# jdm365/SuffixArray

Measured on AMD Instinct MI355X. Metric: sa_build_chars_per_s, higher is better.
Workload: dtype u8 text / u32 narrow keys / u32 suffix indices / i64 output

## Files before the change

suffixarray_amd/csrc/radix_narrow.hpp:

```cpp
#pragma once
#include "radix_sort.hpp"
#include <vector>

namespace sa {

constexpr int NARROW_MAX_PASSES = 6;
constexpr int SEG_ITEMS = 24;

struct SegPlan {
    u32 bstart[RADIX + 1];
    u32 tprefix[RADIX + 1];
    u32 cfirst[NCHUNK + 1];
};

__global__ __launch_bounds__(256) void seg_plan_kernel(const u32* __restrict__ hist_top, u32 tile, SegPlan* __restrict__ plan) {
    __shared__ uint2 s_w[4];
    __shared__ u32 s_tp[RADIX + 1];
    const int d = threadIdx.x;
    u32 size = 0;
#pragma unroll
    for (int c = 0; c < NCHUNK; ++c) size += hist_top[c * RADIX + d];
    const u32 tiles = (u32)(((u64)size + tile - 1) / tile);
    uint2 tot;
    const uint2 ex = block_scan_excl<4>(make_uint2(size, tiles), make_uint2(0, 0), ScanSum{}, s_w, &tot);
// ... 796 lines not shown
    template <typename K>
    int persist_grid(K kernel, int block, int slot, u32 nsub, u32* grid) {
        if (!local_grid[slot]) {
            int dev = 0, cus = 0, per_cu = 0;
            SA_HIP_CHECK(hipGetDevice(&dev));
            SA_HIP_CHECK(hipDeviceGetAttribute(&cus, hipDeviceAttributeMultiprocessorCount, dev));
            SA_HIP_CHECK(hipOccupancyMaxActiveBlocksPerMultiprocessor(&per_cu, reinterpret_cast<const void*>(kernel), block, 0));
            local_grid[slot] = (u32)((per_cu > 0 ? per_cu : 1) * (cus > 0 ? cus : 1));
        }
        const u32 g = local_grid_force ? local_grid_force : local_grid[slot];
        *grid = g < nsub ? g : nsub;
        return 0;
    }
    bool split_flags_done = false;
    int split_items = 28;
    static size_t hist_bytes() { return (size_t)NARROW_MAX_PASSES * RADIX * RADIX * sizeof(u32); }
    int init() {
        SA_HIP_CHECK(hipMalloc(&plan, sizeof(SegPlan)));
        SA_HIP_CHECK(hipMalloc(&hist, hist_bytes()));
        SA_HIP_CHECK(hipMalloc(&base, (size_t)RADIX * RADIX * sizeof(u32)));
        SA_HIP_CHECK(hipMalloc(&tickets, (size_t)NARROW_MAX_PASSES * NCHUNK * sizeof(u32)));
        SA_HIP_CHECK(hipMalloc(&map_dev, sizeof(CodeMap)));
        SA_HIP_CHECK(hipMalloc(&split_hist, split_table_bytes()));
        SA_HIP_CHECK(hipMalloc(&split_base, split_table_bytes()));
        SA_HIP_CHECK(hipMalloc(&split_cursor, split_table_bytes()));
        SA_HIP_CHECK(hipMalloc(&top_cursor, (size_t)RADIX * TOP_CURSOR_STRIDE * sizeof(u32)));
        SA_HIP_CHECK(hipMalloc(&split_sub, (split_sub_words() + 16) * sizeof(u32)));
        SA_HIP_CHECK(hipHostMalloc(reinterpret_cast<void**>(&host_word), 64, hipHostMallocDefault));
        if (const char* e = diag_env("SA_HIP_SPLIT")) split_enabled = atoi(e) != 0;
        if (const char* e = diag_env("SA_HIP_TOP_CLAIMS")) top_claims = atoi(e) != 0;
        if (const char* e = diag_env("SA_HIP_LOCAL_BIG")) local_big = atoi(e) != 0;
        if (const char* e = diag_env("SA_HIP_LOCAL_PERSIST")) local_persist = atoi(e) != 0;
        if (const char* e = diag_env("SA_HIP_LOCAL_GRID")) { const int v = atoi(e); local_grid_force = v > 0 ? (u32)v : 0u; }
        if (const char* e = diag_env("SA_HIP_SPLIT_FLAGS")) split_flags = atoi(e) != 0;
        if (const char* e = diag_env("SA_HIP_LOCAL_BINS")) local_bin_bits = (atoi(e) == 11) ? 11 : 12;
        if (const char* e = diag_env("SA_HIP_SPLIT_ITEMS")) { const int v = atoi(e); split_items = (v == 24 || v == 28) ? v : 32; }
        if (const char* e = diag_env("SA_HIP_SPLIT_CAP")) { const int v = atoi(e); if (v >= 64 && v <= (int)LOCAL_CAP) split_cap = (u32)v; }
        return 0;
    }
    void destroy() {
        if (plan) (void)hipFree(plan);
        if (hist) (void)hipFree(hist);
        if (base) (void)hipFree(base);
        if (tickets) (void)hipFree(tickets);
        if (map_dev) (void)hipFree(map_dev);
        if (split_hist) (void)hipFree(split_hist);
        if (split_base) (void)hipFree(split_base);
        if (split_cursor) (void)hipFree(split_cursor);
        if (top_cursor) (void)hipFree(top_cursor);
        if (split_sub) (void)hipFree(split_sub);
        if (host_word) (void)hipHostFree(host_word);
        map_dev = nullptr;
        plan = nullptr; hist = nullptr; base = nullptr; tickets = nullptr;
        split_hist = split_base = split_sub = split_cursor = top_cursor = nullptr; host_word = nullptr;
    }
};

inline bool narrow_sort_applies(const RadixWorkspace& ws, u64 n, int begin_bit) {
    return ws.block == 512 && begin_bit >= 24 && begin_bit < 56 && n >= (1u << 22) &&
           n / ws.tile() + RADIX + 1 <= ws.max_tiles;
}

struct TextSource {
    const u8* text;
    int b, k0;
};
// ... 88 lines not shown
            a.keys_out32 = reinterpret_cast<u32*>(keysB); a.narrow_shift = begin_bit;
            if ((rc = ws.timer.start(stream, 1))) return rc;
            hipLaunchKernelGGL((radix_onesweep_kernel<512, 0, true>), dim3(g.tiles), dim3(512), 0, stream, a);
            if ((rc = ws.timer.stop(stream, (u64)n * 16u))) return rc;
            ws.pass_records += n; ws.pass_bytes += (u64)n * 16u; ws.passes += 1;
        }
    }
    const u32 seg_tile_n = 512u * SEG_ITEMS;
    const u32 flat_max = n / seg_tile_n + 1 + RADIX;
    const u32 split_tile_n = 512u * (u32)nw.split_items;
    const u32 split_flat_max = n / split_tile_n + 1 + RADIX;
    hipLaunchKernelGGL(seg_plan_kernel, dim3(1), dim3(256), 0, stream, ws.hist(0), try_split ? split_tile_n : seg_tile_n, nw.plan);
    nw.split_used = false;
    nw.split_flags_done = false;
    nw.split_max_seen = 0;
    if (try_split) {
        const int hb = (lo_bits - LOCAL_BIN_BITS < SPLIT_BITS) ? lo_bits - LOCAL_BIN_BITS : SPLIT_BITS;
        SA_HIP_CHECK(hipMemsetAsync(nw.split_hist, 0, NarrowWorkspace::split_table_bytes(), stream));
        SA_HIP_CHECK(hipMemsetAsync(nw.split_levels_dev(), 0, 16 * sizeof(u32), stream));
        const u32 tpb = 4;
        if (nw.split_items == 32)
            hipLaunchKernelGGL((split_hist_kernel<512, 32>), dim3(div_up(split_flat_max, tpb)), dim3(512), 0, stream,
                               reinterpret_cast<const u32*>(keysB), nw.plan, lo_bits - hb, (1u << hb) - 1u, nw.split_hist, tpb);
        else if (nw.split_items == 28)
            hipLaunchKernelGGL((split_hist_kernel<512, 28>), dim3(div_up(split_flat_max, tpb)), dim3(512), 0, stream,
                               reinterpret_cast<const u32*>(keysB), nw.plan, lo_bits - hb, (1u << hb) - 1u, nw.split_hist, tpb);
        else
            hipLaunchKernelGGL((split_hist_kernel<512, 24>), dim3(div_up(split_flat_max, tpb)), dim3(512), 0, stream,
                               reinterpret_cast<const u32*>(keysB), nw.plan, lo_bits - hb, (1u << hb) - 1u, nw.split_hist, tpb);
        hipLaunchKernelGGL(split_levels_kernel, dim3(RADIX), dim3(SPLIT_NB), 0, stream, (const u32*)nw.split_hist, hb, nw.split_levels_dev());
        SA_HIP_CHECK(hipMemcpyAsync(nw.host_word, nw.split_levels_dev(), 16 * sizeof(u32), hipMemcpyDeviceToHost, stream));
        SA_HIP_CHECK(hipStreamSynchronize(stream));
        int rb = -1;
        bool big = nw.local_big;
        if (!big)
            for (int k = 1; k <= hb; ++k)
                if (nw.host_word[k] <= nw.split_cap) { rb = k; break; }
        if (rb < 0 && nw.split_cap == LOCAL_CAP) {
            for (int k = 1; k <= hb; ++k)
                if (nw.host_word[k] <= LOCAL_CAP_BIG && lo_bits - k >= 12) { rb = k; big = true; break; }
            if (rb < 0) big = false;
        }
        nw.split_max_seen = nw.host_word[rb > 0 ? rb : hb];
        if (rb > 0) {
            const int rest_bits = lo_bits - rb;
            const int dshift = lo_bits - rb;
            const u32 dmask = (1u << rb) - 1u;
            hipLaunchKernelGGL(split_scan_kernel, dim3(RADIX), dim3(SPLIT_NB), 0, stream, (const u32*)nw.split_hist, nw.plan, hb, rb,
                               nw.split_base, nw.split_sub);
            SA_HIP_CHECK(hipMemsetAsync(nw.split_cursor, 0, NarrowWorkspace::split_table_bytes(), stream));
            if (++ws.epoch >= (1u << 30)) {
                SA_HIP_CHECK(hipMemsetAsync(ws.status, 0, (size_t)ws.max_tiles * RADIX * sizeof(u64), stream));
                ws.epoch = 1;
            }
            SplitPassArgs a;
            a.keys_in = reinterpret_cast<const u32*>(keysB); a.vals_in = valsB;
            a.keys_out = reinterpret_cast<u32*>(keysA); a.vals_out = valsA;
            a.plan = nw.plan; a.shift = dshift; a.mask = dmask; a.digit_base = nw.split_base;
            a.ticket = nw.tickets; a.cursor = nw.split_cursor;
            if ((rc = ws.timer.start(stream, 2))) return rc;
            if (nw.split_items == 32) hipLaunchKernelGGL((seg_split_kernel<512, 32>), dim3(split_flat_max), dim3(512), 0, stream, a);
            else if (nw.split_items == 28) hipLaunchKernelGGL((seg_split_kernel<512, 28>), dim3(split_flat_max), dim3(512), 0, stream, a);
            else hipLaunchKernelGGL((seg_split_kernel<512, 24>), dim3(split_flat_max), dim3(512), 0, stream, a);
            if ((rc = ws.timer.stop(stream, (u64)n * 16u))) return rc;
            ws.pass_records += n; ws.pass_bytes += (u64)n * 16u; ws.passes += 1;
            LocalArgs l;
            l.keys_in = reinterpret_cast<const u32*>(keysA); l.vals_in = valsA;
            l.keys_out = reinterpret_cast<u32*>(keysB); l.vals_out = valsB; l.vals_out64 = vals_res64;
            l.sub = nw.split_sub;
            const int bb = (big || (rest_bits >= 12 && nw.local_bin_bits == 12)) ? 12 : 11;
            l.bin_shift = rest_bits - bb;
            l.dstat = ws.dstat;
            const u64 local_bytes = (u64)n * 16u + (vals_res64 ? (u64)n * 8u : 0u);
            nw.split_flags_done = false;
            l.dir = DirArgs{}; l.counts = nullptr; l.lite = LiteArgs{}; l.lo_shift = begin_bit; l.rb = rb; l.n = n;
            bool with_flags = false;
            if (nw.split_flags && flags_req && flags_req->prepare) {
                const int fr = flags_req->prepare(flags_req->ctx, (u32)RADIX << rb, &l);
                if (fr < 0) return fr;
                with_flags = (fr == 0) && l.dir.dir && l.dir.dbits >= 8 + rb && l.dir.dbits - 8 - rb <= bb && l.dir.dbits - 8 <= lo_bits;
            }
            if ((rc = ws.timer.start(stream, 3))) return rc;
            const u32 nsub = (u32)RADIX << rb;
            const dim3 lgrid(nsub), lblock(big ? LOCAL_BLOCK_BIG : LOCAL_BLOCK);
            if (nw.local_persist) {
                const int slot = big ? (with_flags ? 0 : 1) : 2 + (with_flags ? 0 : 1) + (bb == 12 ? 0 : 2);
                u32 pg = 0;
                auto go = [&](auto kernel) -> int {
                    if ((rc = nw.persist_grid(kernel, (int)lblock.x, slot, nsub, &pg))) return rc;
                    hipLaunchKernelGGL(kernel, dim3(pg), lblock, 0, stream, l, (const u32*)nw.split_sub, nsub, nw.tickets + NCHUNK, LOCAL_RUN);
                    return 0;
                };
                if (big) rc = with_flags ? go(local_persist_kernel<12, true, LOCAL_BLOCK_BIG>) : go(local_persist_kernel<12, false, LOCAL_BLOCK_BIG>);
                else if (with_flags) rc = (bb == 12) ? go(local_persist_kernel<12, true>) : go(local_persist_kernel<11, true>);
                else rc = (bb == 12) ? go(local_persist_kernel<12, false>) : go(local_persist_kernel<11, false>);
                if (rc) return rc;
            } else if (big) {
                if (with_flags) hipLaunchKernelGGL((local_finish_kernel<12, true, LOCAL_BLOCK_BIG>), lgrid, lblock, 0, stream, l);
                else hipLaunchKernelGGL((local_finish_kernel<12, false, LOCAL_BLOCK_BIG>), lgrid, lblock, 0, stream, l);
            } else if (with_flags) {
                if (bb == 12) hipLaunchKernelGGL((local_finish_kernel<12, true>), lgrid, lblock, 0, stream, l);
                else hipLaunchKernelGGL((local_finish_kernel<11, true>), lgrid, lblock, 0, stream, l);
            } else {
                if (bb == 12) hipLaunchKernelGGL((local_finish_kernel<12, false>), lgrid, lblock, 0, stream, l);
                else hipLaunchKernelGGL((local_finish_kernel<11, false>), lgrid, lblock, 0, stream, l);
            }
            nw.split_flags_done = with_flags;
            nw.split_big = big;
            if ((rc = ws.timer.stop(stream, local_bytes))) return rc;
            ws.pass_records += n; ws.pass_bytes += local_bytes; ws.passes += 1;
            SA_HIP_CHECK(hipGetLastError());
            if (diag_env("SA_HIP_SPLIT_DEBUG")) {
                const u32 nsub = (u32)RADIX << rb;
                std::vector<u32> sub(nsub + 1), k1(n), k2(n), v2(n), bst(RADIX + 1);
                SA_HIP_CHECK(hipStreamSynchronize(stream));
                SA_HIP_CHECK(hipMemcpy(sub.data(), nw.split_sub, (size_t)(nsub + 1) * 4, hipMemcpyDeviceToHost));
                SA_HIP_CHECK(hipMemcpy(k1.data(), keysA, (size_t)n * 4, hipMemcpyDeviceToHost));
                SA_HIP_CHECK(hipMemcpy(k2.data(), keysB, (size_t)n * 4, hipMemcpyDeviceToHost));
                SA_HIP_CHECK(hipMemcpy(v2.data(), valsB, (size_t)n * 4, hipMemcpyDeviceToHost));
                SA_HIP_CHECK(hipMemcpy(bst.data(), nw.plan->bstart, (size_t)(RADIX + 1) * 4, hipMemcpyDeviceToHost));
                u64 bad_sub = 0, bad_split = 0, bad_sorted = 0, bad_mono = 0;
                u32 first_split = ~0u, first_sorted = ~0u;
                for (u32 i = 0; i < nsub; ++i) {
                    if (sub[i] > sub[i + 1] || sub[i + 1] > n) { ++bad_mono; continue; }
                    if ((i & (((u32)1 << rb) - 1)) == 0 && sub[i] != bst[i >> rb]) ++bad_sub;
                    for (u32 j = sub[i]; j < sub[i + 1]; ++j) {
                        if (((k1[j] >> dshift) & dmask) != (i & dmask)) { ++bad_split; if (first_split == ~0u) first_split = j; }
                        if (j > sub[i] && (k2[j - 1] > k2[j] || (k2[j - 1] == k2[j] && v2[j - 1] >= v2[j]))) { ++bad_sorted; if (first_sorted == ~0u) first_sorted = j; }
                    }
                }
                fprintf(stderr, "[sa_hip] split debug: n=%u rb=%d hb=%d nsub=%u sub[0]=%u sub[last]=%u | table: %llu not monotone, %llu off the bucket starts | split pass: %llu records in the wrong group (first %u) | local pass: %llu out of order (first %u)\n",
                        n, rb, hb, nsub, sub[0], sub[nsub], (unsigned long long)bad_mono, (unsigned long long)bad_sub, (unsigned long long)bad_split, first_split,
                        (unsigned long long)bad_sorted, first_sorted);
            }
            nw.split_used = true;
            nw.split_rb = rb;
            *keys_res = reinterpret_cast<u64*>(keysB);
            *vals_res = valsB;
            return 0;
        }
    }
    if (optimistic) {
        SA_HIP_CHECK(hipMemsetAsync(ws.tickets(), 0, NCHUNK * sizeof(u32), stream));
        if (++ws.epoch >= (1u << 30)) {
            SA_HIP_CHECK(hipMemsetAsync(ws.status, 0, (size_t)ws.max_tiles * RADIX * sizeof(u64), stream));
            ws.epoch = 1;
        }
        if ((rc = launch_text_top(false))) return rc;
    }
    if (try_split && split_tile_n != seg_tile_n)
        hipLaunchKernelGGL(seg_plan_kernel, dim3(1), dim3(256), 0, stream, ws.hist(0), seg_tile_n, nw.plan);
    SA_HIP_CHECK(hipMemsetAsync(nw.hist, 0, NarrowWorkspace::hist_bytes(), stream));
    {
        const u32 tpb = 4;
        const u32 mask0 = (1u << ((np == 1) ? lo_bits : RADIX_BITS)) - 1u;
// ... 44 lines not shown
```

suffixarray_amd/csrc/radix_split.hpp:

```cpp
#pragma once
#include "flags_common.hpp"

namespace sa {

#ifndef SA_ABL
#define SA_ABL 0
#endif
constexpr int SPLIT_BITS = 10;
constexpr int SPLIT_NB = 1 << SPLIT_BITS;
constexpr u32 LOCAL_CAP = 8192;
constexpr int LOCAL_BLOCK = 512;
constexpr int LOCAL_ITEMS = (int)(LOCAL_CAP / LOCAL_BLOCK);
constexpr u32 LOCAL_CAP_BIG = 16384;
constexpr int LOCAL_BLOCK_BIG = 1024;
constexpr u32 LOCAL_RUN = 8;
constexpr int LOCAL_BIN_BITS = 11;
constexpr int SPLIT_HIST_COPIES = 4;

template <int BLOCK, int ITEMS>
__global__ __launch_bounds__(BLOCK) void split_hist_kernel(const u32* __restrict__ keys, const SegPlan* __restrict__ plan, int shift,
                                                           u32 mask, u32* __restrict__ hist, u32 tiles_per_block) {
    constexpr u32 TILE = BLOCK * ITEMS;
    constexpr int CS = SPLIT_NB + 1;
    __shared__ u32 s_h[SPLIT_HIST_COPIES * CS];
    __shared__ u32 s_t[RADIX + 1];
    for (int i = threadIdx.x; i <= RADIX; i += BLOCK) s_t[i] = plan->tprefix[i];
    for (int i = threadIdx.x; i < SPLIT_HIST_COPIES * CS; i += BLOCK) s_h[i] = 0;
    __syncthreads();
    const u32 F = s_t[RADIX];
    const u32 f_lo = blockIdx.x * tiles_per_block;
    const u32 f_hi = (f_lo + tiles_per_block < F) ? f_lo + tiles_per_block : F;
    if (f_lo >= f_hi) return;
    u32* my = s_h + (threadIdx.x & (SPLIT_HIST_COPIES - 1)) * CS;
    auto flush = [&](u32 bucket) {
        sync_lds();
        for (int d = threadIdx.x; d < SPLIT_NB; d += BLOCK) {
            u32 v = 0;
#pragma unroll
            for (int k = 0; k < SPLIT_HIST_COPIES; ++k) { v += s_h[k * CS + d]; s_h[k * CS + d] = 0; }
            if (v) atomicAdd(&hist[bucket * SPLIT_NB + d], v);
        }
        sync_lds();
    };
    u32 cur = seg_bucket_of(s_t, f_lo);
    for (u32 f = f_lo; f < f_hi; ++f) {
        const u32 b = seg_bucket_of(s_t, f);
        if (b != cur) { flush(cur); cur = b; }
        const u32 start = plan->bstart[b] + ((f - s_t[b]) * TILE);
        const u32 end = plan->bstart[b + 1];
        const u32 len = (end - start) < TILE ? (end - start) : TILE;
        if (len == TILE) {
            u32 k[ITEMS];
#pragma unroll
            for (int j = 0; j < ITEMS; ++j) k[j] = keys[start + j * BLOCK + threadIdx.x];
#pragma unroll
            for (int j = 0; j < ITEMS; ++j) atomicAdd(&my[(k[j] >> shift) & mask], 1u);
        } else {
            for (u32 l = threadIdx.x; l < len; l += BLOCK) atomicAdd(&my[(keys[start + l] >> shift) & mask], 1u);
        }
    }
    flush(cur);
}

__global__ __launch_bounds__(SPLIT_NB) void split_levels_kernel(const u32* __restrict__ hist, int hb, u32* __restrict__ levels) {
    __shared__ u32 s_p[SPLIT_NB + 1];
    __shared__ u32 s_w[SPLIT_NB / WAVE];
    const int b = blockIdx.x, d = threadIdx.x, lane = d & 63, w = d >> 6;
    const u32 c = hist[b * SPLIT_NB + d];
    s_p[d + 1] = block_scan_excl<SPLIT_NB / WAVE>(c, 0u, ScanSum{}, s_w) + c;
    if (d == 0) s_p[0] = 0;
    __syncthreads();
    __shared__ u32 s_lv[SPLIT_BITS + 1][SPLIT_NB / WAVE];
    for (int k = 0; k <= hb; ++k) {
        const int g = hb - k;
        u32 v = 0;
        if (d < (1 << k)) v = s_p[(d + 1) << g] - s_p[d << g];
#pragma unroll
        for (int o = 32; o > 0; o >>= 1) { const u32 t = __shfl_down(v, o); v = t > v ? t : v; }
        if (lane == 0) s_lv[k][w] = v;
    }
    __syncthreads();
    if (d <= hb) {
        u32 v = 0;
        for (int i = 0; i < SPLIT_NB / WAVE; ++i) v = s_lv[d][i] > v ? s_lv[d][i] : v;
        if (v) atomicMax(&levels[d], v);
    }
}

__global__ __launch_bounds__(SPLIT_NB) void split_scan_kernel(const u32* __restrict__ hist, const SegPlan* __restrict__ plan, int hb, int rb,
                                                              u32* __restrict__ base, u32* __restrict__ sub) {
    __shared__ u32 s_w[SPLIT_NB / WAVE];
    const int b = blockIdx.x, d = threadIdx.x;
    const u32 run = plan->bstart[b] + block_scan_excl<SPLIT_NB / WAVE>(hist[b * SPLIT_NB + d], 0u, ScanSum{}, s_w);
    const int g = hb - rb;
    u32 out = 0;
    if (d < (1 << hb) && (d & ((1 << g) - 1)) == 0) {
        out = run;
        sub[((u32)b << rb) + (u32)(d >> g)] = run;
    }
    __shared__ u32 s_o[SPLIT_NB];
    s_o[d] = 0;
    __syncthreads();
    if (d < (1 << hb) && (d & ((1 << g) - 1)) == 0) s_o[d >> g] = out;
    __syncthreads();
    base[b * SPLIT_NB + d] = s_o[d];
    if (d == 0 && b == RADIX - 1) sub[(u32)RADIX << rb] = plan->bstart[RADIX];
}

struct SplitPassArgs {
    const u32* keys_in;
    const u32* vals_in;
    u32* keys_out;
    u32* vals_out;
    const SegPlan* plan;
    int shift;
    u32 mask;
    const u32* digit_base;
    u32* ticket;
    u32* cursor;
};

template <bool FULL, int BLOCK, int ITEMS>
__device__ __forceinline__ void split_tile(const SplitPassArgs& a, const u32 bucket, const u32 start, const u32 tile_n,
                                           u32* s_keys, u32* s_cnt, u32* s_gdelta, u32* s_wsum) {
    static_assert(SPLIT_NB == 2 * BLOCK, "two bins per thread");
    const int tid = threadIdx.x, lane = tid & 63, wave = tid >> 6;
    const u32 woff = (u32)wave * (WAVE * ITEMS) + lane;

    const uint2 dbase = *reinterpret_cast<const uint2*>(a.digit_base + (size_t)bucket * SPLIT_NB + 2 * tid);

    u32 key[ITEMS];
    const u32* kin = a.keys_in + start;
#pragma unroll
    for (int j = 0; j < ITEMS; ++j) {
        const u32 p = woff + j * WAVE;
        key[j] = (FULL || p < tile_n) ? kin[p] : 0u;
    }
    u32 pos[ITEMS];
#pragma unroll
    for (int j = 0; j < ITEMS; ++j) {
        const u32 d = (key[j] >> a.shift) & a.mask;
        pos[j] = atomicAdd(&s_cnt[(FULL || (woff + j * WAVE) < tile_n) ? d : (u32)SPLIT_NB], 1u);
    }
    sync_lds();
// ... 9 lines not shown
    const u32 incl = wave_scan_incl(tot, ScanSum{});
    if (lane == 63) s_wsum[wave] = incl;
    __syncthreads();
    u32 excl = incl - tot;
    for (int i = 0; i < wave; ++i) excl += s_wsum[i];
    *reinterpret_cast<uint2*>(s_cnt + 2 * tid) = make_uint2(excl, excl + c.x);
    __syncthreads();

#pragma unroll
    for (int j = 0; j < ITEMS; ++j) {
        pos[j] += s_cnt[(key[j] >> a.shift) & a.mask];
        if (FULL || (woff + j * WAVE) < tile_n) s_keys[pos[j]] = key[j];
    }
    __syncthreads();

    *reinterpret_cast<uint2*>(s_gdelta + 2 * tid) = make_uint2(dbase.x + claim0 - excl, dbase.y + claim1 - (excl + c.x));
    __syncthreads();

    static_assert(ITEMS % 2 == 0 && BLOCK * ITEMS <= 65536, "positions packed as 16-bit pairs");
    u32 pp[ITEMS / 2];
#pragma unroll
    for (int j = 0; j < ITEMS / 2; ++j) pp[j] = pos[2 * j] | (pos[2 * j + 1] << 16);
    u32 gidx[ITEMS];
#pragma unroll
    for (int k = 0; k < ITEMS; ++k) {
        const u32 p = k * BLOCK + tid;
        if (FULL || p < tile_n) {
            const u32 kk = s_keys[p];
            gidx[k] = s_gdelta[(kk >> a.shift) & a.mask] + p;
            a.keys_out[gidx[k]] = kk;
        }
    }
    u32 val[ITEMS];
    const u32* vin = a.vals_in + start;
#pragma unroll
    for (int j = 0; j < ITEMS; ++j) {
        const u32 p = woff + j * WAVE;
        val[j] = (FULL || p < tile_n) ? vin[p] : 0u;
    }
    __syncthreads();
    u32* s_vals = s_keys;
#pragma unroll
    for (int j = 0; j < ITEMS; ++j)
        if (FULL || (woff + j * WAVE) < tile_n) s_vals[(pp[j >> 1] >> ((j & 1) * 16)) & 0xFFFFu] = val[j];
    __syncthreads();
#pragma unroll
    for (int k = 0; k < ITEMS; ++k) {
        const u32 p = k * BLOCK + tid;
        if (FULL || p < tile_n) a.vals_out[gidx[k]] = s_vals[p];
    }
}

template <int BLOCK, int ITEMS>
__global__ __launch_bounds__(BLOCK, 4) void seg_split_kernel(SplitPassArgs a) {
    constexpr u32 TILE = BLOCK * ITEMS;
    __shared__ __attribute__((aligned(16))) u32 s_keys[TILE];
    __shared__ __attribute__((aligned(16))) u32 s_cnt[SPLIT_NB + 4];
    __shared__ __attribute__((aligned(16))) u32 s_gdelta[SPLIT_NB];
    __shared__ u32 s_wsum[BLOCK / WAVE];
    __shared__ u32 s_t[RADIX + 1];
    __shared__ u32 s_b[RADIX + 1];
    __shared__ u32 s_c[NCHUNK + 1];
    __shared__ u32 s_flat;

    const int tid = threadIdx.x;
    u32 home = 0, t_home = 0;
    if (tid == 0) {
        home = xcc_id();
// ... 6 lines not shown
    if (tid == 0) {
        u32 flat = 0xFFFFFFFFu;
        if (t_home < s_c[home + 1] - s_c[home]) flat = s_c[home] + t_home;
        for (int k = 1; k < NCHUNK && flat == 0xFFFFFFFFu; ++k) {
            const u32 c = (home + k) & (NCHUNK - 1);
            const u32 cnt = s_c[c + 1] - s_c[c];
            if (cnt == 0) continue;
            const u32 t = atomicAdd(&a.ticket[c], 1u);
            if (t < cnt) flat = s_c[c] + t;
        }
        s_flat = flat;
    }
    __syncthreads();
    const u32 flat = s_flat;
    if (flat == 0xFFFFFFFFu) return;
    const u32 bucket = seg_bucket_of(s_t, flat);
    const u32 first_flat = s_t[bucket];
    const u32 start = s_b[bucket] + (flat - first_flat) * TILE;
    const u32 rest = s_b[bucket + 1] - start;
    if (rest >= TILE) split_tile<true, BLOCK, ITEMS>(a, bucket, start, TILE, s_keys, s_cnt, s_gdelta, s_wsum);
    else split_tile<false, BLOCK, ITEMS>(a, bucket, start, rest, s_keys, s_cnt, s_gdelta, s_wsum);
}

struct LocalArgs {
    const u32* keys_in;
    const u32* vals_in;
    u32* keys_out;
    u32* vals_out;
    int64_t* vals_out64;
    const u32* sub;
    int bin_shift;
    DeviceStatus* dstat;
    DirArgs dir;
    uint2* counts;
    LiteArgs lite;
    int lo_shift;
    int rb;
    u32 n;
};

struct LocalFlagsRequest {
    int (*prepare)(void* ctx, u32 nsub, LocalArgs* l) = nullptr;
    void* ctx = nullptr;
};

template <int BB, bool FLAGS, int BLOCK, bool PERSIST, typename Mid>
__device__ __forceinline__ void local_finish_sub(const LocalArgs& a, const u32 sb, const u32 s, const u32 m, u32 (&key)[LOCAL_ITEMS],
                                                 u32 (&val)[LOCAL_ITEMS], u64* s_rec, u32* s_cw, u32* s_wsum, Mid&& mid) {
    constexpr int ITEMS = LOCAL_ITEMS;
    constexpr int NB = 1 << BB, WORDS = NB / 2, WPT = WORDS / BLOCK;
    const int tid = threadIdx.x, lane = tid & 63, wave = tid >> 6;
    const int g2 = FLAGS ? a.dir.dbits - 8 - a.rb : 0;
    const u32 dfirst = FLAGS ? (sb << g2) : 0u;
    const u32 nd = FLAGS ? (1u << g2) : 0u;
// ... 115 lines not shown
                const u32 kn = (u32)__builtin_amdgcn_update_dpp((int)~k, (int)k, 0x101, 0xF, 0xF, false);
                tmask |= (kn == k && p + 1 < m) ? (1u << j) : 0u;
            }
        }
    }
    if (FLAGS) {
        while (tmask) {
            const u32 j = (u32)__builtin_ctz(tmask);
            tmask &= tmask - 1u;
            stage_pair(j * BLOCK + (u32)tid);
        }
    }
}

template <int BLOCK>
__device__ __forceinline__ void local_load(const LocalArgs& a, const u32 s, const u32 m, u32 (&key)[LOCAL_ITEMS], u32 (&val)[LOCAL_ITEMS]) {
    const u32* kin = a.keys_in + s;
    const u32* vin = a.vals_in + s;
#pragma unroll
    for (int j = 0; j < LOCAL_ITEMS; ++j) {
        const u32 p = (u32)j * BLOCK + threadIdx.x;
        key[j] = 0; val[j] = 0;
        if ((u32)j * BLOCK < m && p < m) { key[j] = kin[p]; val[j] = vin[p]; }
    }
}

template <bool FLAGS, int BLOCK>
__device__ __forceinline__ bool local_short_sub(const LocalArgs& a, const u32 sb, const u32 s, const u32 m, const u32 cap) {
    if (m == 0) {
        if (FLAGS && !(SA_ABL & 8)) {
            const int g2 = a.dir.dbits - 8 - a.rb;
            const u32 dfirst = sb << g2, nd = 1u << g2;
            for (u32 e = threadIdx.x; e < nd; e += BLOCK) a.dir.dir[dfirst + e] = s;
        }
        return true;
    }
    if (m > cap) {
        if (threadIdx.x == 0) __hip_atomic_store(&a.dstat->error, 1u, __ATOMIC_RELAXED, __HIP_MEMORY_SCOPE_AGENT);
        return true;
    }
    if (!FLAGS && m == 1) {
        if (threadIdx.x == 0) {
            const u32 k = a.keys_in[s], v = a.vals_in[s];
            a.keys_out[s] = k; a.vals_out[s] = v;
            if (a.vals_out64) a.vals_out64[s] = (int64_t)v;
        }
        return true;
    }
    return false;
}

template <int BB, bool FLAGS, int BLOCK = LOCAL_BLOCK>
__global__ __launch_bounds__(BLOCK, 4) void local_finish_kernel(LocalArgs a) {
    constexpr u32 CAP = (u32)BLOCK * LOCAL_ITEMS;
    constexpr int NB = 1 << BB, WORDS = NB / 2, WPT = WORDS / BLOCK;
    static_assert(WPT >= 1 && WPT * BLOCK == WORDS, "the scan covers the counters exactly");
    static_assert(CAP < 65536, "16-bit counters and starts");
    __shared__ __attribute__((aligned(16))) u64 s_rec[CAP + 2];
    __shared__ __attribute__((aligned(16))) u32 s_cw[WORDS + 4];
    __shared__ u32 s_wsum[BLOCK / WAVE];
    const u32 sb = blockIdx.x;
    const u32 s = a.sub[sb];
    const u32 m = a.sub[sb + 1] - s;
    if (FLAGS && threadIdx.x == 0 && sb == gridDim.x - 1) a.dir.dir[1u << a.dir.dbits] = a.n;
    if (local_short_sub<FLAGS, BLOCK>(a, sb, s, m, CAP)) return;
#pragma unroll
    for (int i = 0; i < WPT; ++i) s_cw[WPT * threadIdx.x + i] = 0;
    __syncthreads();
    u32 key[LOCAL_ITEMS], val[LOCAL_ITEMS];
    local_load<BLOCK>(a, s, m, key, val);
    local_finish_sub<BB, FLAGS, BLOCK, false>(a, sb, s, m, key, val, s_rec, s_cw, s_wsum, [] {});
}

__device__ __forceinline__ u32 wave_lower_bound(const u32* __restrict__ sub, const u32 nsub, const u64 t) {
    const u32 lane = threadIdx.x & 63u;
    u32 lo = 0, hi = nsub;
    while (lo < hi) {
        const u32 step = (hi - lo + 63u) / 64u;
        const u32 i = lo + lane * step;
        const u32 c = (u32)__popcll(__ballot(i < hi && (u64)sub[i] < t));
        if (c == 0) break;
        const u32 nlo = lo + (c - 1u) * step + 1u;
        hi = (lo + c * step < hi) ? lo + c * step : hi;
        lo = nlo;
    }
// ... 1 lines not shown
}

template <int BB, bool FLAGS, int BLOCK = LOCAL_BLOCK>
__global__ __launch_bounds__(BLOCK, 4) void local_persist_kernel(LocalArgs a, const u32* __restrict__ sub, u32 nsub, u32* ticket, u32 run) {
    constexpr u32 CAP = (u32)BLOCK * LOCAL_ITEMS;
    constexpr int NB = 1 << BB, WORDS = NB / 2, WPT = WORDS / BLOCK;
    static_assert(WPT >= 1 && WPT * BLOCK == WORDS, "the scan covers the counters exactly");
    static_assert(CAP < 65536, "16-bit counters and starts");
    static_assert(BLOCK >= (NCHUNK - 1) * WAVE, "a wave per region bound");
    __shared__ __attribute__((aligned(16))) u64 s_rec[CAP + 2];
    __shared__ __attribute__((aligned(16))) u32 s_cw[WORDS + 4];
    __shared__ u32 s_wsum[BLOCK / WAVE];
    __shared__ u32 s_reg[NCHUNK + 1];
    __shared__ u32 s_run[2];
    const int tid = threadIdx.x;
    {
        const u32 v = (u32)(tid >> 6);
        if (v + 1 < (u32)NCHUNK) {
            const u32 b = wave_lower_bound(sub, nsub, (u64)(v + 1) * sub[nsub] / NCHUNK);
            if ((tid & 63) == 0) s_reg[v + 1] = b;
        }
        if (tid == 0) { s_reg[0] = 0; s_reg[NCHUNK] = nsub; }
    }
#pragma unroll
    for (int i = 0; i < WPT; ++i) s_cw[WPT * tid + i] = 0;
    __syncthreads();
    const u32 home = xcc_id() & (NCHUNK - 1);
    u32 lo = 0, hi = 0;
    auto grab = [&] {
        if (tid == 0) {
// ... 15 lines not shown
    auto next = [&](u32 i, u32& s, u32& m) -> u32 {
        for (;; ++i) {
            if (i >= hi) {
                grab();
                if (lo >= hi) return nsub;
                i = lo;
            }
            s = sub[i]; m = sub[i + 1] - s;
            if (FLAGS && tid == 0 && i == nsub - 1) a.dir.dir[1u << a.dir.dbits] = a.n;
            if (!local_short_sub<FLAGS, BLOCK>(a, i, s, m, CAP)) return i;
        }
    };
    u32 key[LOCAL_ITEMS], val[LOCAL_ITEMS];
    u32 s = 0, m = 0;
    u32 i = next(0, s, m);
    if (i < nsub) local_load<BLOCK>(a, s, m, key, val);
    while (i < nsub) {
        u32 ns = 0, nm = 0;
        const u32 nx = next(i + 1, ns, nm);
        local_finish_sub<BB, FLAGS, BLOCK, true>(a, i, s, m, key, val, s_rec, s_cw, s_wsum, [&] {
            if (nx < nsub) local_load<BLOCK>(a, ns, nm, key, val);
        });
        i = nx; s = ns; m = nm;
    }
}

}
```

Before: 65.75 billion.

## Add sampled-histogram split pass writing into fixed-stride slack slots with exact fallback

For large inputs, the split pass now builds its histogram from a sampled subset of tiles and sets the split level from a conservative statistical lower bound. It then scatters records into fixed-capacity, fixed-stride slots in a separate slack buffer, so the exact prefix-scan base is no longer needed. Actual group sizes are recovered afterwards from the cursors. If any slot overflows, the local kernels exit early and the whole split reruns in exact mode. This cuts the histogram read of the keys and the scan, but adds a large extra allocation, a host sync to check for overflow, and the risk of paying for the work twice.

```diff
diff --git a/suffixarray_amd/csrc/radix_narrow.hpp b/suffixarray_amd/csrc/radix_narrow.hpp
--- a/suffixarray_amd/csrc/radix_narrow.hpp
+++ b/suffixarray_amd/csrc/radix_narrow.hpp
@@ -834,6 +834,32 @@
     }
     bool split_flags_done = false;
     int split_items = 28;
+    int split_slack = -1;
+    u32 slack_pad = SPLIT_SLACK_PAD;
+    size_t slack_max_mb = SPLIT_SLACK_MAX_MB;
+    u32* slack_keys = nullptr;
+    u32* slack_vals = nullptr;
+    size_t slack_entries = 0;
+    bool split_slack_used = false;
+    bool split_overflowed = false;
+    bool ensure_slack(size_t entries) {
+        if (entries <= slack_entries) return true;
+        if (entries * 2 * sizeof(u32) > slack_max_mb * ((size_t)1 << 20)) return false;
+        release_slack();
+        if (hipMalloc(&slack_keys, entries * sizeof(u32)) != hipSuccess || hipMalloc(&slack_vals, entries * sizeof(u32)) != hipSuccess) {
+            (void)hipGetLastError();
+            release_slack();
+            return false;
+        }
+        slack_entries = entries;
+        return true;
+    }
+    void release_slack() {
+        if (slack_keys) (void)hipFree(slack_keys);
+        if (slack_vals) (void)hipFree(slack_vals);
+        slack_keys = slack_vals = nullptr;
+        slack_entries = 0;
+    }
     static size_t hist_bytes() { return (size_t)NARROW_MAX_PASSES * RADIX * RADIX * sizeof(u32); }
     int init() {
         SA_HIP_CHECK(hipMalloc(&plan, sizeof(SegPlan)));
@@ -855,6 +881,9 @@
         if (const char* e = diag_env("SA_HIP_SPLIT_FLAGS")) split_flags = atoi(e) != 0;
         if (const char* e = diag_env("SA_HIP_LOCAL_BINS")) local_bin_bits = (atoi(e) == 11) ? 11 : 12;
         if (const char* e = diag_env("SA_HIP_SPLIT_ITEMS")) { const int v = atoi(e); split_items = (v == 24 || v == 28) ? v : 32; }
+        if (const char* e = diag_env("SA_HIP_SPLIT_SLACK")) split_slack = atoi(e) != 0 ? 1 : 0;
+        if (const char* e = diag_env("SA_HIP_SPLIT_SLACK_PAD")) { const int v = atoi(e); if (v >= 0 && v <= 4096) slack_pad = (u32)v & ~31u; }
+        if (const char* e = diag_env("SA_HIP_SPLIT_SLACK_MAX_MB")) { const long long v = atoll(e); if (v >= 0) slack_max_mb = (size_t)v; }
         if (const char* e = diag_env("SA_HIP_SPLIT_CAP")) { const int v = atoi(e); if (v >= 64 && v <= (int)LOCAL_CAP) split_cap = (u32)v; }
         return 0;
     }
@@ -870,6 +899,7 @@
         if (top_cursor) (void)hipFree(top_cursor);
         if (split_sub) (void)hipFree(split_sub);
         if (host_word) (void)hipHostFree(host_word);
+        release_slack();
         map_dev = nullptr;
         plan = nullptr; hist = nullptr; base = nullptr; tickets = nullptr;
         split_hist = split_base = split_sub = split_cursor = top_cursor = nullptr; host_word = nullptr;
@@ -988,21 +1018,27 @@
     nw.split_used = false;
     nw.split_flags_done = false;
     nw.split_max_seen = 0;
-    if (try_split) {
+    nw.split_slack_used = false;
+    nw.split_overflowed = false;
+    enum { SPLIT_TAKEN, SPLIT_DECLINED, SPLIT_EXACT };
+    auto split_attempt = [&](const bool slack, int* outcome) -> int {
+        *outcome = SPLIT_DECLINED;
         const int hb = (lo_bits - LOCAL_BIN_BITS < SPLIT_BITS) ? lo_bits - LOCAL_BIN_BITS : SPLIT_BITS;
         SA_HIP_CHECK(hipMemsetAsync(nw.split_hist, 0, NarrowWorkspace::split_table_bytes(), stream));
         SA_HIP_CHECK(hipMemsetAsync(nw.split_levels_dev(), 0, 16 * sizeof(u32), stream));
-        const u32 tpb = 4;
+        const u32 hstride = slack ? SPLIT_SAMPLE : 1u;
+        const u32 tpb = 4 * hstride;
         if (nw.split_items == 32)
             hipLaunchKernelGGL((split_hist_kernel<512, 32>), dim3(div_up(split_flat_max, tpb)), dim3(512), 0, stream,
-                               reinterpret_cast<const u32*>(keysB), nw.plan, lo_bits - hb, (1u << hb) - 1u, nw.split_hist, tpb);
+                               reinterpret_cast<const u32*>(keysB), nw.plan, lo_bits - hb, (1u << hb) - 1u, nw.split_hist, tpb, hstride);
         else if (nw.split_items == 28)
             hipLaunchKernelGGL((split_hist_kernel<512, 28>), dim3(div_up(split_flat_max, tpb)), dim3(512), 0, stream,
-                               reinterpret_cast<const u32*>(keysB), nw.plan, lo_bits - hb, (1u << hb) - 1u, nw.split_hist, tpb);
+                               reinterpret_cast<const u32*>(keysB), nw.plan, lo_bits - hb, (1u << hb) - 1u, nw.split_hist, tpb, hstride);
         else
             hipLaunchKernelGGL((split_hist_kernel<512, 24>), dim3(div_up(split_flat_max, tpb)), dim3(512), 0, stream,
-                               reinterpret_cast<const u32*>(keysB), nw.plan, lo_bits - hb, (1u << hb) - 1u, nw.split_hist, tpb);
-        hipLaunchKernelGGL(split_levels_kernel, dim3(RADIX), dim3(SPLIT_NB), 0, stream, (const u32*)nw.split_hist, hb, nw.split_levels_dev());
+                               reinterpret_cast<const u32*>(keysB), nw.plan, lo_bits - hb, (1u << hb) - 1u, nw.split_hist, tpb, hstride);
+        hipLaunchKernelGGL(split_levels_kernel, dim3(RADIX), dim3(SPLIT_NB), 0, stream, (const u32*)nw.split_hist, hb, nw.split_levels_dev(),
+                           slack ? (const SegPlan*)nw.plan : (const SegPlan*)nullptr, SPLIT_SAMPLE_Z);
         SA_HIP_CHECK(hipMemcpyAsync(nw.host_word, nw.split_levels_dev(), 16 * sizeof(u32), hipMemcpyDeviceToHost, stream));
         SA_HIP_CHECK(hipStreamSynchronize(stream));
         int rb = -1;
@@ -1016,32 +1052,54 @@
             if (rb < 0) big = false;
         }
         nw.split_max_seen = nw.host_word[rb > 0 ? rb : hb];
-        if (rb > 0) {
+        if (rb <= 0) return 0;
+        const u32 slot_cap = big ? LOCAL_CAP_BIG : nw.split_cap;
+        const u32 slot_stride = (big ? LOCAL_CAP_BIG : LOCAL_CAP) + nw.slack_pad;
+        const u32 nsub = (u32)RADIX << rb;
+        if (slack && (big || !nw.ensure_slack((size_t)nsub * slot_stride))) { *outcome = SPLIT_EXACT; return 0; }
+        if (slack && diag_env("SA_HIP_DEBUG_ADDR"))
+            fprintf(stderr, "[sa_hip] addr slack_keys=%p slack_vals=%p entries=%zu stride=%u\n", (void*)nw.slack_keys, (void*)nw.slack_vals, nw.slack_entries, slot_stride);
+        {
             const int rest_bits = lo_bits - rb;
             const int dshift = lo_bits - rb;
             const u32 dmask = (1u << rb) - 1u;
-            hipLaunchKernelGGL(split_scan_kernel, dim3(RADIX), dim3(SPLIT_NB), 0, stream, (const u32*)nw.split_hist, nw.plan, hb, rb,
-                               nw.split_base, nw.split_sub);
+            if (!slack)
+                hipLaunchKernelGGL(split_scan_kernel, dim3(RADIX), dim3(SPLIT_NB), 0, stream, (const u32*)nw.split_hist, nw.plan, hb, rb,
+                                   nw.split_base, nw.split_sub);
             SA_HIP_CHECK(hipMemsetAsync(nw.split_cursor, 0, NarrowWorkspace::split_table_bytes(), stream));
             if (++ws.epoch >= (1u << 30)) {
                 SA_HIP_CHECK(hipMemsetAsync(ws.status, 0, (size_t)ws.max_tiles * RADIX * sizeof(u64), stream));
                 ws.epoch = 1;
             }
+            u32* const mid_keys = slack ? nw.slack_keys : reinterpret_cast<u32*>(keysA);
+            u32* const mid_vals = slack ? nw.slack_vals : valsA;
             SplitPassArgs a;
             a.keys_in = reinterpret_cast<const u32*>(keysB); a.vals_in = valsB;
-            a.keys_out = reinterpret_cast<u32*>(keysA); a.vals_out = valsA;
+            a.keys_out = mid_keys; a.vals_out = mid_vals;
             a.plan = nw.plan; a.shift = dshift; a.mask = dmask; a.digit_base = nw.split_base;
             a.ticket = nw.tickets; a.cursor = nw.split_cursor;
+            a.rb = rb; a.stride = slot_stride; a.cap = slot_cap; a.overflow = nw.split_levels_dev() + SPLIT_INFO_OVERFLOW;
             if ((rc = ws.timer.start(stream, 2))) return rc;
-            if (nw.split_items == 32) hipLaunchKernelGGL((seg_split_kernel<512, 32>), dim3(split_flat_max), dim3(512), 0, stream, a);
-            else if (nw.split_items == 28) hipLaunchKernelGGL((seg_split_kernel<512, 28>), dim3(split_flat_max), dim3(512), 0, stream, a);
-            else hipLaunchKernelGGL((seg_split_kernel<512, 24>), dim3(split_flat_max), dim3(512), 0, stream, a);
+            if (slack) {
+                if (nw.split_items == 32) hipLaunchKernelGGL((seg_split_kernel<512, 32, true>), dim3(split_flat_max), dim3(512), 0, stream, a);
+                else if (nw.split_items == 28) hipLaunchKernelGGL((seg_split_kernel<512, 28, true>), dim3(split_flat_max), dim3(512), 0, stream, a);
+                else hipLaunchKernelGGL((seg_split_kernel<512, 24, true>), dim3(split_flat_max), dim3(512), 0, stream, a);
+            } else {
+                if (nw.split_items == 32) hipLaunchKernelGGL((seg_split_kernel<512, 32>), dim3(split_flat_max), dim3(512), 0, stream, a);
+                else if (nw.split_items == 28) hipLaunchKernelGGL((seg_split_kernel<512, 28>), dim3(split_flat_max), dim3(512), 0, stream, a);
+                else hipLaunchKernelGGL((seg_split_kernel<512, 24>), dim3(split_flat_max), dim3(512), 0, stream, a);
+            }
             if ((rc = ws.timer.stop(stream, (u64)n * 16u))) return rc;
             ws.pass_records += n; ws.pass_bytes += (u64)n * 16u; ws.passes += 1;
+            if (slack)
+                hipLaunchKernelGGL(split_sizes_kernel, dim3(RADIX), dim3(SPLIT_NB), 0, stream, (const u32*)nw.split_cursor, nw.plan, rb,
+                                   nw.split_sub, nw.split_levels_dev());
             LocalArgs l;
-            l.keys_in = reinterpret_cast<const u32*>(keysA); l.vals_in = valsA;
+            l.keys_in = mid_keys; l.vals_in = mid_vals;
             l.keys_out = reinterpret_cast<u32*>(keysB); l.vals_out = valsB; l.vals_out64 = vals_res64;
             l.sub = nw.split_sub;
+            l.in_stride = slack ? slot_stride : 0u;
+            l.overflow = slack ? nw.split_levels_dev() + SPLIT_INFO_OVERFLOW : nullptr;
             const int bb = (big || (rest_bits >= 12 && nw.local_bin_bits == 12)) ? 12 : 11;
             l.bin_shift = rest_bits - bb;
             l.dstat = ws.dstat;
@@ -1050,12 +1108,11 @@
             l.dir = DirArgs{}; l.counts = nullptr; l.lite = LiteArgs{}; l.lo_shift = begin_bit; l.rb = rb; l.n = n;
             bool with_flags = false;
             if (nw.split_flags && flags_req && flags_req->prepare) {
-                const int fr = flags_req->prepare(flags_req->ctx, (u32)RADIX << rb, &l);
+                const int fr = flags_req->prepare(flags_req->ctx, nsub, &l);
                 if (fr < 0) return fr;
                 with_flags = (fr == 0) && l.dir.dir && l.dir.dbits >= 8 + rb && l.dir.dbits - 8 - rb <= bb && l.dir.dbits - 8 <= lo_bits;
             }
             if ((rc = ws.timer.start(stream, 3))) return rc;
-            const u32 nsub = (u32)RADIX << rb;
             const dim3 lgrid(nsub), lblock(big ? LOCAL_BLOCK_BIG : LOCAL_BLOCK);
             if (nw.local_persist) {
                 const int slot = big ? (with_flags ? 0 : 1) : 2 + (with_flags ? 0 : 1) + (bb == 12 ? 0 : 2);
@@ -1079,40 +1136,67 @@
                 if (bb == 12) hipLaunchKernelGGL((local_finish_kernel<12, false>), lgrid, lblock, 0, stream, l);
                 else hipLaunchKernelGGL((local_finish_kernel<11, false>), lgrid, lblock, 0, stream, l);
             }
+            if ((rc = ws.timer.stop(stream, slack ? 0u : local_bytes))) return rc;
+            if (slack) {
+                SA_HIP_CHECK(hipMemcpyAsync(nw.host_word + SPLIT_INFO_OVERFLOW, nw.split_levels_dev() + SPLIT_INFO_OVERFLOW, 2 * sizeof(u32),
+                                            hipMemcpyDeviceToHost, stream));
+                SA_HIP_CHECK(hipStreamSynchronize(stream));
+                if (nw.host_word[SPLIT_INFO_OVERFLOW]) {
+                    nw.split_overflowed = true;
+                    nw.split_max_seen = 0;
+                    SA_HIP_CHECK(hipMemsetAsync(nw.tickets, 0, (size_t)NARROW_MAX_PASSES * NCHUNK * sizeof(u32), stream));
+                    *outcome = SPLIT_EXACT;
+                    return 0;
+                }
+                nw.split_max_seen = nw.host_word[SPLIT_INFO_MAX];
+                ws.timer.kind_bytes[3] += local_bytes;
+            }
             nw.split_flags_done = with_flags;
             nw.split_big = big;
-            if ((rc = ws.timer.stop(stream, local_bytes))) return rc;
             ws.pass_records += n; ws.pass_bytes += local_bytes; ws.passes += 1;
             SA_HIP_CHECK(hipGetLastError());
             if (diag_env("SA_HIP_SPLIT_DEBUG")) {
-                const u32 nsub = (u32)RADIX << rb;
-                std::vector<u32> sub(nsub + 1), k1(n), k2(n), v2(n), bst(RADIX + 1);
+                const size_t mid_n = slack ? (size_t)nsub * slot_stride : (size_t)n;
+                std::vector<u32> sub(nsub + 1), k1(mid_n), k2(n), v2(n), bst(RADIX + 1);
                 SA_HIP_CHECK(hipStreamSynchronize(stream));
                 SA_HIP_CHECK(hipMemcpy(sub.data(), nw.split_sub, (size_t)(nsub + 1) * 4, hipMemcpyDeviceToHost));
-                SA_HIP_CHECK(hipMemcpy(k1.data(), keysA, (size_t)n * 4, hipMemcpyDeviceToHost));
+                SA_HIP_CHECK(hipMemcpy(k1.data(), mid_keys, mid_n * 4, hipMemcpyDeviceToHost));
                 SA_HIP_CHECK(hipMemcpy(k2.data(), keysB, (size_t)n * 4, hipMemcpyDeviceToHost));
                 SA_HIP_CHECK(hipMemcpy(v2.data(), valsB, (size_t)n * 4, hipMemcpyDeviceToHost));
                 SA_HIP_CHECK(hipMemcpy(bst.data(), nw.plan->bstart, (size_t)(RADIX + 1) * 4, hipMemcpyDeviceToHost));
-                u64 bad_sub = 0, bad_split = 0, bad_sorted = 0, bad_mono = 0;
+                u64 bad_sub = 0, bad_split = 0, bad_sorted = 0, bad_mono = 0, bad_slot = 0;
                 u32 first_split = ~0u, first_sorted = ~0u;
                 for (u32 i = 0; i < nsub; ++i) {
                     if (sub[i] > sub[i + 1] || sub[i + 1] > n) { ++bad_mono; continue; }
                     if ((i & (((u32)1 << rb) - 1)) == 0 && sub[i] != bst[i >> rb]) ++bad_sub;
+                    if (slack && sub[i + 1] - sub[i] > slot_cap) { ++bad_slot; continue; }
                     for (u32 j = sub[i]; j < sub[i + 1]; ++j) {
-                        if (((k1[j] >> dshift) & dmask) != (i & dmask)) { ++bad_split; if (first_split == ~0u) first_split = j; }
+                        const size_t at = slack ? (size_t)i * slot_stride + (j - sub[i]) : (size_t)j;
+                        if (((k1[at] >> dshift) & dmask) != (i & dmask)) { ++bad_split; if (first_split == ~0u) first_split = j; }
                         if (j > sub[i] && (k2[j - 1] > k2[j] || (k2[j - 1] == k2[j] && v2[j - 1] >= v2[j]))) { ++bad_sorted; if (first_sorted == ~0u) first_sorted = j; }
                     }
                 }
-                fprintf(stderr, "[sa_hip] split debug: n=%u rb=%d hb=%d nsub=%u sub[0]=%u sub[last]=%u | table: %llu not monotone, %llu off the bucket starts | split pass: %llu records in the wrong group (first %u) | local pass: %llu out of order (first %u)\n",
-                        n, rb, hb, nsub, sub[0], sub[nsub], (unsigned long long)bad_mono, (unsigned long long)bad_sub, (unsigned long long)bad_split, first_split,
-                        (unsigned long long)bad_sorted, first_sorted);
+                fprintf(stderr, "[sa_hip] split debug: n=%u rb=%d hb=%d nsub=%u sub[0]=%u sub[last]=%u slack=%d stride=%u | table: %llu not monotone, %llu off the bucket starts, %llu beyond their slot | split pass: %llu records in the wrong group (first %u) | local pass: %llu out of order (first %u)\n",
+                        n, rb, hb, nsub, sub[0], sub[nsub], slack ? 1 : 0, slack ? slot_stride : 0u, (unsigned long long)bad_mono, (unsigned long long)bad_sub,
+                        (unsigned long long)bad_slot, (unsigned long long)bad_split, first_split, (unsigned long long)bad_sorted, first_sorted);
             }
             nw.split_used = true;
             nw.split_rb = rb;
+            nw.split_slack_used = slack;
             *keys_res = reinterpret_cast<u64*>(keysB);
             *vals_res = valsB;
+            *outcome = SPLIT_TAKEN;
             return 0;
         }
+    };
+    if (try_split) {
+        const int hb_max = (lo_bits - LOCAL_BIN_BITS < SPLIT_BITS) ? lo_bits - LOCAL_BIN_BITS : SPLIT_BITS;
+        const bool slack = (nw.split_slack < 0 ? n >= SPLIT_SLACK_MIN_N : nw.split_slack != 0) && !nw.local_big &&
+                           (u64)n <= (u64)nw.split_cap * ((u64)RADIX << hb_max);
+        int outcome = SPLIT_EXACT;
+        if (slack && (rc = split_attempt(true, &outcome))) return rc;
+        if (outcome == SPLIT_EXACT && (rc = split_attempt(false, &outcome))) return rc;
+        if (outcome == SPLIT_TAKEN) return 0;
     }
     if (optimistic) {
         SA_HIP_CHECK(hipMemsetAsync(ws.tickets(), 0, NCHUNK * sizeof(u32), stream));
diff --git a/suffixarray_amd/csrc/radix_split.hpp b/suffixarray_amd/csrc/radix_split.hpp
--- a/suffixarray_amd/csrc/radix_split.hpp
+++ b/suffixarray_amd/csrc/radix_split.hpp
@@ -16,10 +16,18 @@
 constexpr u32 LOCAL_RUN = 8;
 constexpr int LOCAL_BIN_BITS = 11;
 constexpr int SPLIT_HIST_COPIES = 4;
+constexpr u32 SPLIT_SAMPLE = 8;
+constexpr double SPLIT_SAMPLE_Z = 4.0;
+constexpr u32 SPLIT_SLACK_PAD = 0;
+constexpr u32 SPLIT_SLACK_MIN_N = 1u << 25;
+constexpr u32 SPLIT_SLACK_MAX_MB = 20480;
+constexpr u32 SPLIT_SKIP = 0x80000000u;
+constexpr int SPLIT_INFO_OVERFLOW = 12;
+constexpr int SPLIT_INFO_MAX = 13;
 
 template <int BLOCK, int ITEMS>
 __global__ __launch_bounds__(BLOCK) void split_hist_kernel(const u32* __restrict__ keys, const SegPlan* __restrict__ plan, int shift,
-                                                           u32 mask, u32* __restrict__ hist, u32 tiles_per_block) {
+                                                           u32 mask, u32* __restrict__ hist, u32 tiles_per_block, u32 stride) {
     constexpr u32 TILE = BLOCK * ITEMS;
     constexpr int CS = SPLIT_NB + 1;
     __shared__ u32 s_h[SPLIT_HIST_COPIES * CS];
@@ -46,6 +54,7 @@
     for (u32 f = f_lo; f < f_hi; ++f) {
         const u32 b = seg_bucket_of(s_t, f);
         if (b != cur) { flush(cur); cur = b; }
+        if ((f - s_t[b]) % stride) continue;
         const u32 start = plan->bstart[b] + ((f - s_t[b]) * TILE);
         const u32 end = plan->bstart[b + 1];
         const u32 len = (end - start) < TILE ? (end - start) : TILE;
@@ -62,7 +71,8 @@
     flush(cur);
 }
 
-__global__ __launch_bounds__(SPLIT_NB) void split_levels_kernel(const u32* __restrict__ hist, int hb, u32* __restrict__ levels) {
+__global__ __launch_bounds__(SPLIT_NB) void split_levels_kernel(const u32* __restrict__ hist, int hb, u32* __restrict__ levels,
+                                                                const SegPlan* __restrict__ plan, double z) {
     __shared__ u32 s_p[SPLIT_NB + 1];
     __shared__ u32 s_w[SPLIT_NB / WAVE];
     const int b = blockIdx.x, d = threadIdx.x, lane = d & 63, w = d >> 6;
@@ -70,11 +80,17 @@
     s_p[d + 1] = block_scan_excl<SPLIT_NB / WAVE>(c, 0u, ScanSum{}, s_w) + c;
     if (d == 0) s_p[0] = 0;
     __syncthreads();
+    double ratio = 0.0;
+    if (plan && s_p[SPLIT_NB]) ratio = (double)(plan->bstart[b + 1] - plan->bstart[b]) / (double)s_p[SPLIT_NB];
     __shared__ u32 s_lv[SPLIT_BITS + 1][SPLIT_NB / WAVE];
     for (int k = 0; k <= hb; ++k) {
         const int g = hb - k;
         u32 v = 0;
         if (d < (1 << k)) v = s_p[(d + 1) << g] - s_p[d << g];
+        if (plan) {
+            const double low = (double)v - z * sqrt((double)v);
+            v = low > 0.0 ? (u32)(ratio * low) : 0u;
+        }
 #pragma unroll
         for (int o = 32; o > 0; o >>= 1) { const u32 t = __shfl_down(v, o); v = t > v ? t : v; }
         if (lane == 0) s_lv[k][w] = v;
@@ -104,6 +120,19 @@
     if (d < (1 << hb) && (d & ((1 << g) - 1)) == 0) s_o[d >> g] = out;
     __syncthreads();
     base[b * SPLIT_NB + d] = s_o[d];
+    if (d == 0 && b == RADIX - 1) sub[(u32)RADIX << rb] = plan->bstart[RADIX];
+}
+
+__global__ __launch_bounds__(SPLIT_NB) void split_sizes_kernel(const u32* __restrict__ cursor, const SegPlan* __restrict__ plan, int rb,
+                                                               u32* __restrict__ sub, u32* __restrict__ info) {
+    __shared__ u32 s_w[SPLIT_NB / WAVE];
+    const int b = blockIdx.x, d = threadIdx.x;
+    const u32 c = cursor[b * SPLIT_NB + d];
+    const u32 run = plan->bstart[b] + block_scan_excl<SPLIT_NB / WAVE>(c, 0u, ScanSum{}, s_w);
+    if (d < (1 << rb)) sub[((u32)b << rb) + (u32)d] = run;
+    u32 largest = 0;
+    (void)block_scan_excl<SPLIT_NB / WAVE>(c, 0u, ScanMax{}, s_w, &largest);
+    if (d == 0 && largest) atomicMax(&info[SPLIT_INFO_MAX], largest);
     if (d == 0 && b == RADIX - 1) sub[(u32)RADIX << rb] = plan->bstart[RADIX];
 }
 
@@ -118,16 +147,27 @@
     const u32* digit_base;
     u32* ticket;
     u32* cursor;
+    int rb;
+    u32 stride;
+    u32 cap;
+    u32* overflow;
 };
 
-template <bool FULL, int BLOCK, int ITEMS>
+template <bool FULL, int BLOCK, int ITEMS, bool SLACK>
 __device__ __forceinline__ void split_tile(const SplitPassArgs& a, const u32 bucket, const u32 start, const u32 tile_n,
                                            u32* s_keys, u32* s_cnt, u32* s_gdelta, u32* s_wsum) {
     static_assert(SPLIT_NB == 2 * BLOCK, "two bins per thread");
     const int tid = threadIdx.x, lane = tid & 63, wave = tid >> 6;
     const u32 woff = (u32)wave * (WAVE * ITEMS) + lane;
 
-    const uint2 dbase = *reinterpret_cast<const uint2*>(a.digit_base + (size_t)bucket * SPLIT_NB + 2 * tid);
+    uint2 dbase;
+    u32* kout = a.keys_out;
+    u32* vout = a.vals_out;
+    if (SLACK) {
+        dbase = make_uint2(2u * (u32)tid * a.stride, (2u * (u32)tid + 1u) * a.stride);
+        const size_t part = (size_t)(bucket << a.rb) * a.stride;
+        kout += part; vout += part;
+    } else dbase = *reinterpret_cast<const uint2*>(a.digit_base + (size_t)bucket * SPLIT_NB + 2 * tid);
 
     u32 key[ITEMS];
     const u32* kin = a.keys_in + start;
@@ -167,7 +207,14 @@
     }
     __syncthreads();
 
-    *reinterpret_cast<uint2*>(s_gdelta + 2 * tid) = make_uint2(dbase.x + claim0 - excl, dbase.y + claim1 - (excl + c.x));
+    uint2 gd = make_uint2(dbase.x + claim0 - excl, dbase.y + claim1 - (excl + c.x));
+    if (SLACK) {
+        const bool o0 = c.x && claim0 + c.x > a.cap, o1 = c.y && claim1 + c.y > a.cap;
+        if (o0 || o1) __hip_atomic_store(a.overflow, 1u, __ATOMIC_RELAXED, __HIP_MEMORY_SCOPE_AGENT);
+        if (o0) gd.x = SPLIT_SKIP - excl;
+        if (o1) gd.y = SPLIT_SKIP - (excl + c.x);
+    }
+    *reinterpret_cast<uint2*>(s_gdelta + 2 * tid) = gd;
     __syncthreads();
 
     static_assert(ITEMS % 2 == 0 && BLOCK * ITEMS <= 65536, "positions packed as 16-bit pairs");
@@ -181,7 +228,7 @@
         if (FULL || p < tile_n) {
             const u32 kk = s_keys[p];
             gidx[k] = s_gdelta[(kk >> a.shift) & a.mask] + p;
-            a.keys_out[gidx[k]] = kk;
+            if (!SLACK || gidx[k] < SPLIT_SKIP) kout[gidx[k]] = kk;
         }
     }
     u32 val[ITEMS];
@@ -200,11 +247,11 @@
 #pragma unroll
     for (int k = 0; k < ITEMS; ++k) {
         const u32 p = k * BLOCK + tid;
-        if (FULL || p < tile_n) a.vals_out[gidx[k]] = s_vals[p];
-    }
-}
-
-template <int BLOCK, int ITEMS>
+        if ((FULL || p < tile_n) && (!SLACK || gidx[k] < SPLIT_SKIP)) vout[gidx[k]] = s_vals[p];
+    }
+}
+
+template <int BLOCK, int ITEMS, bool SLACK = false>
 __global__ __launch_bounds__(BLOCK, 4) void seg_split_kernel(SplitPassArgs a) {
     constexpr u32 TILE = BLOCK * ITEMS;
     __shared__ __attribute__((aligned(16))) u32 s_keys[TILE];
@@ -241,12 +288,12 @@
     __syncthreads();
     const u32 flat = s_flat;
     if (flat == 0xFFFFFFFFu) return;
-    const u32 bucket = seg_bucket_of(s_t, flat);
+    const u32 bucket = SLACK ? (u32)__builtin_amdgcn_readfirstlane((int)seg_bucket_of(s_t, flat)) : seg_bucket_of(s_t, flat);
     const u32 first_flat = s_t[bucket];
     const u32 start = s_b[bucket] + (flat - first_flat) * TILE;
     const u32 rest = s_b[bucket + 1] - start;
-    if (rest >= TILE) split_tile<true, BLOCK, ITEMS>(a, bucket, start, TILE, s_keys, s_cnt, s_gdelta, s_wsum);
-    else split_tile<false, BLOCK, ITEMS>(a, bucket, start, rest, s_keys, s_cnt, s_gdelta, s_wsum);
+    if (rest >= TILE) split_tile<true, BLOCK, ITEMS, SLACK>(a, bucket, start, TILE, s_keys, s_cnt, s_gdelta, s_wsum);
+    else split_tile<false, BLOCK, ITEMS, SLACK>(a, bucket, start, rest, s_keys, s_cnt, s_gdelta, s_wsum);
 }
 
 struct LocalArgs {
@@ -264,7 +311,13 @@
     int lo_shift;
     int rb;
     u32 n;
+    u32 in_stride;
+    const u32* overflow;
 };
+
+__device__ __forceinline__ u64 local_in_offset(const LocalArgs& a, const u32 sb, const u32 s) {
+    return a.in_stride ? (u64)sb * a.in_stride : (u64)s;
+}
 
 struct LocalFlagsRequest {
     int (*prepare)(void* ctx, u32 nsub, LocalArgs* l) = nullptr;
@@ -410,9 +463,10 @@
 }
 
 template <int BLOCK>
-__device__ __forceinline__ void local_load(const LocalArgs& a, const u32 s, const u32 m, u32 (&key)[LOCAL_ITEMS], u32 (&val)[LOCAL_ITEMS]) {
-    const u32* kin = a.keys_in + s;
-    const u32* vin = a.vals_in + s;
+__device__ __forceinline__ void local_load(const LocalArgs& a, const u32 sb, const u32 s, const u32 m, u32 (&key)[LOCAL_ITEMS], u32 (&val)[LOCAL_ITEMS]) {
+    const u64 in = local_in_offset(a, sb, s);
+    const u32* kin = a.keys_in + in;
+    const u32* vin = a.vals_in + in;
 #pragma unroll
     for (int j = 0; j < LOCAL_ITEMS; ++j) {
         const u32 p = (u32)j * BLOCK + threadIdx.x;
@@ -437,7 +491,8 @@
     }
     if (!FLAGS && m == 1) {
         if (threadIdx.x == 0) {
-            const u32 k = a.keys_in[s], v = a.vals_in[s];
+            const u64 in = local_in_offset(a, sb, s);
+            const u32 k = a.keys_in[in], v = a.vals_in[in];
             a.keys_out[s] = k; a.vals_out[s] = v;
             if (a.vals_out64) a.vals_out64[s] = (int64_t)v;
         }
@@ -455,6 +510,7 @@
     __shared__ __attribute__((aligned(16))) u64 s_rec[CAP + 2];
     __shared__ __attribute__((aligned(16))) u32 s_cw[WORDS + 4];
     __shared__ u32 s_wsum[BLOCK / WAVE];
+    if (a.overflow && *a.overflow) return;
     const u32 sb = blockIdx.x;
     const u32 s = a.sub[sb];
     const u32 m = a.sub[sb + 1] - s;
@@ -464,7 +520,7 @@
     for (int i = 0; i < WPT; ++i) s_cw[WPT * threadIdx.x + i] = 0;
     __syncthreads();
     u32 key[LOCAL_ITEMS], val[LOCAL_ITEMS];
-    local_load<BLOCK>(a, s, m, key, val);
+    local_load<BLOCK>(a, sb, s, m, key, val);
     local_finish_sub<BB, FLAGS, BLOCK, false>(a, sb, s, m, key, val, s_rec, s_cw, s_wsum, [] {});
 }
 
@@ -496,6 +552,7 @@
     __shared__ u32 s_reg[NCHUNK + 1];
     __shared__ u32 s_run[2];
     const int tid = threadIdx.x;
+    if (a.overflow && *a.overflow) return;
     {
         const u32 v = (u32)(tid >> 6);
         if (v + 1 < (u32)NCHUNK) {
@@ -541,12 +598,12 @@
     u32 key[LOCAL_ITEMS], val[LOCAL_ITEMS];
     u32 s = 0, m = 0;
     u32 i = next(0, s, m);
-    if (i < nsub) local_load<BLOCK>(a, s, m, key, val);
+    if (i < nsub) local_load<BLOCK>(a, i, s, m, key, val);
     while (i < nsub) {
         u32 ns = 0, nm = 0;
         const u32 nx = next(i + 1, ns, nm);
         local_finish_sub<BB, FLAGS, BLOCK, true>(a, i, s, m, key, val, s_rec, s_cw, s_wsum, [&] {
-            if (nx < nsub) local_load<BLOCK>(a, ns, nm, key, val);
+            if (nx < nsub) local_load<BLOCK>(a, nx, ns, nm, key, val);
         });
         i = nx; s = ns; m = nm;
     }
```

Measured after the change: 65.87 billion, median of 6. Within noise of the previous version (+0.2%).
